# filodb/FiloDB

Measured on NVIDIA H100. Metric: samples/s scanned+aggregated (rate over 10M series); % HBM roofline, higher is better.
Workload: dtype f64

## Files before the change

### filodb_b200/csrc/capi.cu

```cuda
#include "../../include/filo_b200.h"
#include "kernels.h"
#include "host_util.h"
#include "scan_tile_layout.h"
#include "scan_wp_layout.h"
#include <cub/cub.cuh>
#include <algorithm>
#include <atomic>
#include <chrono>
#include <cmath>
#include <cstdio>
#include <cstdlib>
#include <cstring>
#include <mutex>
#include <string>
#include <thread>
#include <vector>

using namespace filo;

struct filo_ctx {
  int device = 0;
  filo_cfg cfg{};
  cudaStream_t stream = nullptr;
  int sm_count = 132;
// ... 799 lines not shown
  const uint32_t acc_bytes = fused ? align_up((uint32_t)q.T * (moments ? 20u : 12u), 128) : 0;
  const bool need_corr2 = need_corr && t->any_drop;
  uint32_t scratch2 = align_up((uint32_t)t->max_chunks * (uint32_t)CHUNK_DESC_BYTES, 16) +
                      ((uint32_t)t->max_rows + (uint32_t)t->max_chunks * 8u) * 8u * (1u + (t->any_nonconst_ts ? 1u : 0u) + (need_corr2 ? 1u : 0u));
  scratch2 = align_up(scratch2 + 16, 128);
  const uint32_t rec_cap = align_up(t->max_rec_bytes + 16, 128);
  const size_t per_warp2 = v2_smem_per_warp(rec_cap, scratch2, acc_bytes);
  const char* force_env = std::getenv("FILO_KERNEL");
  const std::string force = force_env ? force_env : "";
  const size_t smem_cap = std::min<size_t>(ctx->max_smem_optin, 227 * 1024);
  const bool use_v2 = force != "v1" && t->max_rec_bytes > 0 && per_warp2 * FAST_WARPS + 1024 <= smem_cap;
  const int64_t work = fused ? t->n_items : t->n_series;
  int64_t launches = 0;
  uint8_t* gscratch = nullptr;
  ScanLaunch L{t->d_arena, t->d_rec_off, t->n_series, q, nullptr, 0, 0, d_counters, d_err, 1, s};
  uint32_t rec_cap_used = 0;
  if (use_v2) {
    const size_t cta_smem = per_warp2 * FAST_WARPS + 1024;
    const int ctas_per_sm = (int)std::max<size_t>(1, std::min<size_t>(64 / FAST_WARPS, (size_t)(228 * 1024) / cta_smem));
    L.grid = (int)std::max<int64_t>(1, std::min<int64_t>((work + FAST_WARPS - 1) / FAST_WARPS, (int64_t)ctx->sm_count * ctas_per_sm));
    L.scratch_bytes = scratch2; L.use_smem = 1; rec_cap_used = rec_cap;
  } else {
    uint32_t scratch = align_up((uint32_t)t->max_chunks * (uint32_t)CHUNK_DESC_BYTES, 16) + (uint32_t)t->max_rows * 8u * (need_corr ? 3u : 2u);
    scratch = align_up(scratch + 16, 16);
    const size_t cta_smem = (size_t)(scratch + acc_bytes) * SCAN_WARPS;
    const int use_smem = cta_smem <= std::min<size_t>(ctx->max_smem_optin, 200 * 1024);
    int ctas_per_sm = 16;
    if (use_smem) ctas_per_sm = (int)std::max<size_t>(1, std::min<size_t>(16, (size_t)(220 * 1024) / std::max<size_t>(cta_smem + 1024, 1)));
    L.grid = (int)std::max<int64_t>(1, std::min<int64_t>((work + SCAN_WARPS - 1) / SCAN_WARPS, (int64_t)ctx->sm_count * ctas_per_sm));
    if (!use_smem) CUDA_TRY(ctx, tmp.alloc((void**)&gscratch, (size_t)L.grid * SCAN_WARPS * (scratch + acc_bytes)));
    L.gscratch = gscratch; L.scratch_bytes = scratch; L.use_smem = use_smem;
  }
  const int fn_cls = fn_class_of(fn, q.cumulative, q.long_values);
  const uint64_t wrows = (uint64_t)(q.window / q.step) + 1;
  TileSmem TL{};
  bool use_tile = false;
  if (use_v2 && force != "v2" && fn_cls == CLASS_SUM && t->n_series > 0) {
    TL = tile_layout(t->max_rec_bytes, (uint32_t)t->max_rows, (uint32_t)q.T, (uint32_t)std::min<uint64_t>(2 * wrows, 1u << 20) + 16);
    if (((size_t)TL.total + 1024) * 2 > (size_t)228 * 1024) TL = tile_layout(t->max_rec_bytes, (uint32_t)t->max_rows, (uint32_t)q.T, 16);
    use_tile = (size_t)TL.total + 1024 <= smem_cap;
  }
  WpSmem WL{};
  WpBatchSmem WB{};
  bool use_wp = false, use_wp_batch = false;
  if (use_tile && force != "v3" && wrows <= 4096 && t->max_chunks > 0) {
    const bool alias = wp_max_items((uint32_t)t->max_chunks, (uint32_t)q.T, (uint32_t)wrows) <= 64;
    WL = wp_layout(t->max_rec_bytes, (uint32_t)t->max_rows, (uint32_t)t->max_chunks, (uint32_t)q.T, (uint32_t)wrows, alias);
    WL.warps = (uint32_t)std::min<size_t>(smem_cap / WL.per_warp, alias ? WP_MAX_WARPS_ALIAS : WP_MAX_WARPS);
    const WpSmem WL2 = wp_layout(t->max_rec_bytes, (uint32_t)t->max_rows, (uint32_t)t->max_chunks, (uint32_t)q.T, (uint32_t)wrows, alias, true);
    if (smem_cap / WL2.per_warp >= (size_t)WP_MAX_WARPS) {
      WL = WL2; WL.warps = WP_MAX_WARPS;
      WB = wp_batch_layout(t->max_rec_bytes, (uint32_t)t->max_rows, (uint32_t)t->max_chunks, (uint32_t)q.T, (uint32_t)wrows, alias);
      use_wp_batch = WB.total <= smem_cap;
    }
    use_wp = WL.warps >= 4;
  }
  WpCtrSmem WC{};
  bool use_wp_ctr = false;
  if (use_v2 && force != "v2" && force != "v3" && fn_cls == CLASS_COUNTER && t->n_series > 0 && t->max_chunks > 0 &&
      (!fused || q.T <= TILE_AGG_ACC * TILE_THREADS) && wp_ctr_tile_footprint_ok(t->max_rec_bytes, (uint32_t)t->max_rows, (uint32_t)q.T, smem_cap)) {
    WC = wp_ctr_layout(t->max_rec_bytes, (uint32_t)t->max_rows, (uint32_t)t->max_chunks, (uint32_t)q.T, fused, t->any_nonconst_ts, moments);
    const size_t w = std::min<size_t>((smem_cap - sizeof(TileCtrTab) * (TILE_CTR_TABMAX + 1) - 64) / WC.per_warp, WC.tsr != 0 ? 16 : WP_CTR_MAX_WARPS);
    WC.warps = (uint32_t)w; WC.tab = (uint32_t)(WC.per_warp * w);
    use_wp_ctr = w >= 4;
  }
  auto run_per_series = [&](double* outp) -> int32_t {
    if (use_tile || use_wp_ctr) {
      int64_t* d_list = nullptr; unsigned long long* d_cnt = nullptr;
      CUDA_TRY(ctx, tmp.alloc((void**)&d_list, (size_t)t->n_series * 8));
      CUDA_TRY(ctx, tmp.alloc((void**)&d_cnt, 16));
      CUDA_TRY(ctx, cudaMemsetAsync(d_cnt, 0, 16, s));
      ScanLaunch LT = L;
      static const bool dbg = std::getenv("FILO_DEBUG_SYNC") != nullptr;
      if (use_wp_batch) {
        LT.grid = (int)std::max<int64_t>(1, std::min<int64_t>((t->n_series + WB.B - 1) / WB.B, (int64_t)ctx->sm_count));
        CUDA_TRY(ctx, launch_scan_wp_batch(LT, outp, WB, d_list, d_cnt));
      } else if (use_wp) {
        LT.grid = (int)std::max<int64_t>(1, std::min<int64_t>((t->n_series + WL.warps - 1) / WL.warps, (int64_t)ctx->sm_count));
        CUDA_TRY(ctx, launch_scan_wp(LT, outp, WL, d_list, d_cnt));
      } else if (use_wp_ctr) {
        LT.grid = (int)std::max<int64_t>(1, std::min<int64_t>((t->n_series + WC.warps - 1) / WC.warps, (int64_t)ctx->sm_count));
        CUDA_TRY(ctx, launch_scan_wp_ctr(LT, outp, WC, d_list, d_cnt));
      } else {
        const int ctas_per_sm = ((size_t)TL.total + 1024) * 2 <= (size_t)228 * 1024 ? 2 : 1;
        const int64_t n_tiles = (t->n_series + TILE_NS - 1) / TILE_NS;
        LT.grid = (int)std::max<int64_t>(1, std::min<int64_t>(n_tiles, (int64_t)ctx->sm_count * ctas_per_sm));
        if (dbg) { fprintf(stderr, "[filo] tile kernel fn=%d T=%d grid=%d smem=%u pitch=%u\n", fn, q.T, LT.grid, TL.total, TL.vals_pitch); fflush(stderr); }
        CUDA_TRY(ctx, launch_scan_tile(LT, outp, TL, d_list, d_cnt));
      }
      if (dbg) { CUDA_TRY(ctx, cudaStreamSynchronize(s)); fprintf(stderr, "[filo] tile kernel done\n"); fflush(stderr); }
      ScanLaunch LF = L; LF.list = d_list; LF.list_count = d_cnt;
      CUDA_TRY(ctx, launch_scan_series_v2(LF, outp, rec_cap_used));
      if (dbg) { CUDA_TRY(ctx, cudaStreamSynchronize(s)); fprintf(stderr, "[filo] fallback kernel done\n"); fflush(stderr); }
      launches += 2;
    } else {
      CUDA_TRY(ctx, use_v2 ? launch_scan_series_v2(L, outp, rec_cap_used) : launch_scan_series(L, outp));
      launches += 1;
    }
    return FILO_OK;
  };
  if (stats) CUDA_TRY(ctx, cudaEventRecord(e0, s));
  if (agg == FILO_AGG_NONE) {
    { int32_t rc = run_per_series((double*)d_out_values); if (rc) return rc; }
  } else if (!fused) {
    double* per = nullptr;
    CUDA_TRY(ctx, tmp.alloc((void**)&per, (size_t)t->n_series * q.T * 8));
// ... 559 lines not shown
```

### filodb_b200/csrc/scan_wp.cuh

```cuda
#pragma once
#include "scan_tile.cuh"
#include "scan_wp_layout.h"

namespace filo {

#ifdef FILO_CUSIM
__device__ __forceinline__ uint32_t wp_soff(const void* p) { return (uint32_t)(reinterpret_cast<const uint8_t*>(p) - smem); }
__device__ __forceinline__ uint32_t wp_lds32(uint32_t off) { uint32_t v; std::memcpy(&v, smem + off, 4); return v; }
#else
__device__ __forceinline__ uint32_t wp_soff(const void* p) { return smem_u32(p); }
__device__ __forceinline__ uint32_t wp_lds32(uint32_t off) { uint32_t v; asm volatile("ld.shared.u32 %0, [%1];" : "=r"(v) : "r"(off)); return v; }
#endif

#if defined(FILO_WP_PROF) && !defined(FILO_CUSIM)
__device__ unsigned long long g_wp_prof[32];
#define WPROF_DECL uint32_t wpp_t0 = (uint32_t)clock(), wpp_acc[14] = {0, 0, 0, 0, 0, 0, 0, 0, 0, 0, 0, 0, 0, 0};
#define WPROF(i) { const uint32_t wpp_t1 = (uint32_t)clock(); wpp_acc[i] += wpp_t1 - wpp_t0; wpp_t0 = wpp_t1; }
#define WPROF_COUNT(i) { ++wpp_acc[i]; }
#define WPROF_FLUSH if (lane == 0) { for (int wpp_i = 0; wpp_i < 14; ++wpp_i) atomicAdd(&g_wp_prof[wpp_i], (unsigned long long)wpp_acc[wpp_i]); atomicAdd(&g_wp_prof[15], 1ull); }
#else
#define WPROF_DECL
#define WPROF(i)
#define WPROF_COUNT(i)
#define WPROF_FLUSH
// ... 211 lines not shown
        TileDrops& D = DR[ci];
#pragma unroll
        for (int i = 0; i < 8; ++i) {
          const double cur = nan0(__longlong_as_double((long long)(d[jj][i] ^ pre)));
          if (i < nleft && cur < prevv) {
            const int at = atomicAdd(&D.n, 1);
            if (at < TILE_MAXDROP) { D.pos[at] = 1 + g * 8 + i; D.amt[at] = prevv; }
          }
          prevv = cur;
        }
      }
    }
  }
  for (int ci = 0; any_raw && ci < n; ++ci) {
    const WpChunk& ch = CD[ci];
    if (ch.wire != WIRE_RAW64) continue;
    const uint64_t* src = reinterpret_cast<const uint64_t*>(R + ch.val_off + 8);
    const bool drp = DROPS && ch.dropped;
    for (int r = lane; r < ch.nrows; r += 32) {
      const uint64_t b = src[r];
      reinterpret_cast<uint64_t*>(V)[wp_vidx(ch.rowpos + r)] = b;
      const uint32_t h = (uint32_t)(b >> 32);
      okbits &= h ^ (h << 1);
      if (drp && r > 0) {
        const double cur = nan0(__longlong_as_double((long long)b)), prevv = nan0(__longlong_as_double((long long)src[r - 1]));
        if (cur < prevv) { TileDrops& D = DR[ci]; const int at = atomicAdd(&D.n, 1); if (at < TILE_MAXDROP) { D.pos[at] = r; D.amt[at] = prevv; } }
      }
    }
  }
  if (any_raw) r_done();
  return okbits;
}

constexpr uint32_t WP_FINAL = 0, WP_RAWFIN = 1, WP_JUNC = 2, WP_GAP = 3;
__device__ __forceinline__ int wp_chunk_of(const WpChunk* CD, int n, int k) {
  int ci = -1;
  for (int c = 0; c < n; ++c) if (CD[c].nblk > 0 && k >= CD[c].kT0) ci = c;
  return ci;
}
__device__ __forceinline__ uint32_t wp_class(const WpChunk* CD, int n, int k, uint32_t& jslot) {
  const int ci = wp_chunk_of(CD, n, k);
  jslot = 0;
  if (ci < 0 || k > CD[ci].kT1) return WP_GAP;
  const WpChunk& ch = CD[ci];
  const int i = k - ch.kT0;
  if (i < ch.jzb * WP_R) { jslot = (uint32_t)(ch.joff + i) | (i < ch.hs ? 128u : 0u); return WP_JUNC; }
  return i >= ch.tb * WP_R ? WP_RAWFIN : WP_FINAL;
}
__device__ __forceinline__ int wp_rows_in(const WpChunk& x, int k, int Wr) {
  int lo = x.s0 + k; if (lo < 0) lo = 0; int hi = x.s0 + k + Wr; if (hi > x.nrows - 1) hi = x.nrows - 1;
  return hi - lo + 1;
}

__device__ __forceinline__ void wp_item(const WpChunk* CD, const WpSmem& L, int it, int items, int psi, int& pp, int& op, int& inf) {
  const bool active = it < items;
  int ci = 0;
  if (CD[1].nblk > 0 && it >= CD[1].blk0) ci = 1;
  if (CD[2].nblk > 0 && it >= CD[2].blk0) ci = 2;
  if (CD[3].nblk > 0 && it >= CD[3].blk0) ci = 3;
  const WpChunk& ch = CD[ci];
  const int b = active ? it - ch.blk0 : 0;
  const int k0 = ch.kT0 + WP_R * b;
  pp = ch.vidx0 + 9 * b;
  const bool tojz = b < ch.jzb;
  const bool raw = tojz || b >= ch.tb;
  op = tojz ? (int)WP_OFF_J + 8 * (ch.joff + WP_R * b) : (int)L.out + 8 * (k0 + ((k0 + psi) >> 3));
  int jEnd = !active ? -1 : tojz ? WP_R - 1 : ch.kT1 - k0;
  if (jEnd > WP_R - 1) jEnd = WP_R - 1;
  const int ot = tojz ? 0 : (k0 + psi) & 7;
  inf = (jEnd + 1) | ((raw ? 1 : 0) << 4) | (ot << 5) | (ci << 8) | (k0 << 10);
}

struct WpQuery {
  double fdiv, frcp;
  int64_t S0, E0, lastEnd;
  StepDiv sd;
  __device__ __forceinline__ void init(const QueryParams& q) {
    int64_t winDur = q.inclusive ? q.window : q.window - 1; if (winDur < 0) winDur = 0;
    fdiv = (double)(q.inclusive ? winDur : winDur + 1); frcp = 1.0 / fdiv;
    S0 = q.start - winDur; E0 = q.start;
    lastEnd = q.start + (int64_t)(q.T - 1) * q.step;
    sd.init(q.step);
  }
};
struct WpPlan {
  int64_t m_init = 0, m_end = 0; int m_nrows = -1, m_n = -1, m_wire = -1; bool m_ok = false;
  int dd_dst[2] = {0, 0}, dd_inf[2] = {0, 0}, wi_pp[2] = {0, 0}, wi_op[2] = {0, 0}, wi_inf[2] = {0, 0};
  int gz[3] = {-1, -1, -1}; bool gz_all = true;
  int p_Wr = 0, p_items = 0, p_nfull = 0, p_psi = 0; double p_rcpn = 0.0; bool p_oal = false;
  uint32_t p_cls = 0; uint64_t p_jx = 0;
};

__device__ __forceinline__ bool wp_plan_series(WpPlan& M, bool& regular, bool have, int n, int64_t init, int64_t end_time, int nrows, int vwire,
                                               int grp_base, int ngroups, const QueryParams& q, const WpSmem& L, const WpQuery& Q, WpChunk* CD, int lane) {
  const unsigned FULL = 0xffffffffu;
  const int c = lane;
  const bool samec = !(c < n) || (init == M.m_init && nrows == M.m_nrows && end_time == M.m_end && vwire == M.m_wire);
  const bool same_all = __all_sync(FULL, samec);
  const bool same = M.m_ok && n == M.m_n && same_all;
  const bool miss = regular && !same;
  if (miss) {
    M.m_init = init; M.m_end = end_time; M.m_nrows = nrows; M.m_n = n; M.m_wire = vwire; M.m_ok = false;
    int64_t s0 = 0, e0 = 0;
    if (have) { s0 = Q.sd.ceil_div(Q.S0 - init); e0 = Q.sd.floor_div(Q.E0 - init); }
    const int Wr = (int)(e0 - s0);
    int64_t kT0 = -e0; if (kT0 < 0) kT0 = 0;
    int64_t kT1 = (int64_t)(nrows - 1) - s0; if (kT1 > q.T - 1) kT1 = q.T - 1;
    const bool touch = have && kT0 <= kT1;
    if (!touch) { kT0 = 0x3fffffff; kT1 = -1; }
    const int Wr0 = __shfl_sync(FULL, Wr, 0);
    bool okp = !have || Wr == Wr0;
    if (Wr0 < 8 || (uint32_t)Wr0 + 1 > L.jcap) okp = false;
    const unsigned tm = __ballot_sync(FULL, touch) & 0xfu;
    if (tm != 0) { const unsigned lowbit = tm & (0u - tm); const unsigned filled = tm + lowbit; if ((filled & (filled - 1)) != 0) okp = false; }
    const int64_t kT1p = __shfl_up_sync(FULL, kT1, 1), kT1pp = __shfl_up_sync(FULL, kT1, 2), kT0n = __shfl_down_sync(FULL, kT0, 1);
    const bool prev_t = c > 0 && ((tm >> (c - 1)) & 1u), next_t = c + 1 < WP_MAXC && ((tm >> (c + 1)) & 1u);
    if (touch && c >= 2 && ((tm >> (c - 2)) & 1u) && !(kT1pp < kT0)) okp = false;
    int64_t ownLo = kT0, ownHi = kT1;
    if (touch && prev_t && kT1p + 1 > ownLo) ownLo = kT1p + 1;
    if (touch && next_t && kT0n - 1 < ownHi) ownHi = kT0n - 1;
    const int hs = touch ? (int)(ownLo - kT0) : 0;
    const int nblk = touch ? (int)((kT1 - kT0 + WP_R) / WP_R) : 0;
    const int jzb = (hs + WP_R - 1) / WP_R;
    const int tb = (touch && ownHi < kT1) ? (int)((ownHi + 1 - kT0) / WP_R) : nblk;
    if (touch && jzb > tb) okp = false;
    int blk0, items, joff, jtot;
    { const int a0 = __shfl_sync(FULL, nblk, 0), a1 = __shfl_sync(FULL, nblk, 1), a2 = __shfl_sync(FULL, nblk, 2), a3 = __shfl_sync(FULL, nblk, 3);
      blk0 = (c > 0 ? a0 : 0) + (c > 1 ? a1 : 0) + (c > 2 ? a2 : 0); items = a0 + a1 + a2 + a3; }
    { const int z = jzb * WP_R;
      const int a0 = __shfl_sync(FULL, z, 0), a1 = __shfl_sync(FULL, z, 1), a2 = __shfl_sync(FULL, z, 2), a3 = __shfl_sync(FULL, z, 3);
      joff = (c > 0 ? a0 : 0) + (c > 1 ? a1 : 0) + (c > 2 ? a2 : 0); jtot = a0 + a1 + a2 + a3; }
    if ((uint32_t)jtot > L.jcap) okp = false;
    if (L.alias && items > 64) okp = false;
    const int fr = touch ? (int)(s0 + kT0) : 0;
    int rowpos = 0;
    {
      int base = 0;
#pragma unroll
      for (int cc = 0; cc < WP_MAXC; ++cc) {
        int x;
        if (cc == 0) { x = fr < 0 ? -fr : ((8 - (fr & 7)) & 7); }
        else { x = base + ((-(base + fr)) & 7); }
        if (c == cc) rowpos = x;
        const int nb = __shfl_sync(FULL, x + nrows + Wr0, cc);
        base = nb;
      }
    }
    const int pend = __shfl_sync(FULL, rowpos + nrows, n > 0 ? n - 1 : 0) + Wr0 + 8;
    if ((uint32_t)(pend + (pend >> 3) + 2) > L.vcap) okp = false;
    if (!__all_sync(FULL, okp)) regular = false;
    if (regular) {
      if (c < WP_MAXC) {
        WpChunk& d = CD[c];
        d.kT0 = (int)kT0; d.kT1 = (int)kT1; d.ownLo = (int)ownLo; d.ownHi = (int)ownHi; d.blk0 = blk0; d.nblk = nblk;
        d.vidx0 = wp_vidx(rowpos + fr); d.rowpos = rowpos; d.nrows = nrows; d.s0 = (int)s0; d.e0 = (int)e0; d.joff = joff; d.hs = hs; d.jzb = jzb; d.tb = tb;
      }
      { const int first_t = tm ? __ffs((int)tm) - 1 : 0;
        M.p_psi = (-(int)__shfl_sync(FULL, (int)(touch ? kT0 : 0), first_t)) & 7;
        M.p_oal = __all_sync(FULL, !touch || (((int)kT0 + M.p_psi) & 7) == 0); }
      M.p_Wr = Wr0; M.p_items = items; M.p_nfull = Wr0 + 1; M.p_rcpn = 1.0 / (double)(Wr0 + 1);
      __syncwarp();
      {
        int tot = 0;
        M.gz[0] = M.gz[1] = M.gz[2] = -1;
        for (int g = 0; g <= n; ++g) {
          const int g0 = g == 0 ? 0 : CD[g - 1].rowpos + CD[g - 1].nrows;
          const int g1 = g == n ? pend : CD[g].rowpos;
#pragma unroll
          for (int u = 0; u < 3; ++u) { const int i = u * 32 + lane - tot; if (i >= 0 && i < g1 - g0) M.gz[u] = wp_vidx(g0 + i); }
          tot += g1 - g0;
        }
        M.gz_all = tot <= 96;
      }
      {
        uint32_t cls = 0; uint64_t jx = 0; int nj = 0;
#pragma unroll 1
        for (int m = 0; m < 16 && lane + 32 * m < q.T; ++m) {
          uint32_t js;
          const uint32_t code = wp_class(CD, n, lane + 32 * m, js);
          cls |= code << (2 * m);
          if (code == WP_JUNC) { jx |= (uint64_t)js << (8 * nj); ++nj; }
        }
        M.p_cls = cls; M.p_jx = jx;
      }
      {
        const int gb1 = __shfl_sync(FULL, have ? grp_base : 0x7fffffff, 1), gb2 = __shfl_sync(FULL, have ? grp_base : 0x7fffffff, 2),
                  gb3 = __shfl_sync(FULL, have ? grp_base : 0x7fffffff, 3);
#pragma unroll
        for (int jj = 0; jj < 2; ++jj) {
          const int slot = jj * 32 + lane;
          const bool active = slot < ngroups;
          const int ci = active ? (slot >= gb1 ? 1 : 0) + (slot >= gb2 ? 1 : 0) + (slot >= gb3 ? 1 : 0) : 0;
          const int gbc = ci == 0 ? 0 : ci == 1 ? gb1 : ci == 2 ? gb2 : gb3;
          const int g = active ? slot - gbc : 0;
          const int pq = CD[ci].rowpos + 1 + g * 8;
          M.dd_dst[jj] = wp_vidx(pq);
          M.dd_inf[jj] = (active ? 1 : 0) | (ci << 1) | ((pq & 7) << 3) | (g << 8);
        }
#pragma unroll
        for (int X = 0; X < 2; ++X) wp_item(CD, L, X * 32 + lane, items, M.p_psi, M.wi_pp[X], M.wi_op[X], M.wi_inf[X]);
      }
      M.m_ok = true;
    }
  }
  return miss;
}

__device__ __forceinline__ void wp_zero_rows(double* V, const WpChunk* CD, int n, const WpPlan& M, int lane) {
  if (M.gz_all) {
#pragma unroll
    for (int u = 0; u < 3; ++u) if (M.gz[u] >= 0) V[M.gz[u]] = 0.0;
  } else {
    const int pend = CD[n - 1].rowpos + CD[n - 1].nrows + M.p_Wr + 8;
    for (int g = 0; g <= n; ++g) {
      const int g0 = g == 0 ? 0 : CD[g - 1].rowpos + CD[g - 1].nrows;
      const int g1 = g == n ? pend : CD[g].rowpos;
      for (int pz = g0 + lane; pz < g1; pz += 32) V[wp_vidx(pz)] = 0.0;
    }
  }
}

template <int FN>
__device__ __forceinline__ void wp_window_blocks(const double* V, uint8_t* wb, const WpChunk* CD, const WpSmem& L, const WpPlan& M, const WpQuery& Q,
                                                 int lane) {
  const int psi = M.p_psi;
  const int Wr = M.p_Wr;
  for (int it0 = 0; it0 < M.p_items; it0 += 64) {
    int ipp[2], iop[2], iinf[2];
#pragma unroll
    for (int X = 0; X < 2; ++X) {
      if (it0 == 0) { ipp[X] = M.wi_pp[X]; iop[X] = M.wi_op[X]; iinf[X] = M.wi_inf[X]; }
      else wp_item(CD, L, it0 + X * 32 + lane, M.p_items, psi, ipp[X], iop[X], iinf[X]);
    }
    const double* pp[2]; double* op[2]; int jEnd[2], ot[2]; bool rawm[2];
#pragma unroll
    for (int X = 0; X < 2; ++X) {
      pp[X] = V + ipp[X]; op[X] = reinterpret_cast<double*>(wb + iop[X]);
      jEnd[X] = (iinf[X] & 15) - 1; rawm[X] = (iinf[X] >> 4) & 1; ot[X] = (iinf[X] >> 5) & 7;
    }
    double a[WP_R], bb[WP_R];
    wp_block_pair(pp[0], pp[1], Wr, a, bb);
    __syncwarp();
#pragma unroll
    for (int X = 0; X < 2; ++X) {
      const double dv = rawm[X] ? 1.0 : Q.fdiv, rc = rawm[X] ? 1.0 : Q.frcp, sc = rawm[X] ? 1.0 : 1000.0;
#pragma unroll
      for (int j = 0; j < WP_R; ++j) {
        const double raw = X ? bb[j] : a[j];
        int nn = 1;
        if (FN == FN_AVG || FN == FN_COUNT) {
          const WpChunk& ch = CD[(iinf[X] >> 8) & 3];
          int lo = ch.s0 + (iinf[X] >> 10) + j; const int hi0 = lo + Wr; if (lo < 0) lo = 0;
          const int hi = hi0 > ch.nrows - 1 ? ch.nrows - 1 : hi0;
          nn = hi - lo + 1;
        }
        const double fin = wp_finish<FN>(raw, nn, dv, rc, sc, M.p_nfull, M.p_rcpn, rawm[X]);
        if (X) bb[j] = fin; else a[j] = fin;
      }
    }
    if (M.p_oal) {
#pragma unroll
      for (int j = 0; j < WP_R; ++j) { if (j <= jEnd[0]) op[0][j] = a[j]; if (j <= jEnd[1]) op[1][j] = bb[j]; }
    } else {
#pragma unroll
      for (int j = 0; j < WP_R; ++j) {
        if (j <= jEnd[0]) op[0][j + ((ot[0] + j) >> 3)] = a[j];
        if (j <= jEnd[1]) op[1][j + ((ot[1] + j) >> 3)] = bb[j];
      }
    }
  }
  __syncwarp();
}

template <int FN, bool STAGE = false>
__device__ __forceinline__ void wp_finish_store(double* __restrict__ out, int64_t s, const QueryParams& q, double* O, const double* J,
                                                const WpChunk* CD, int n, const WpPlan& M, const WpQuery& Q, int lane) {
  const double NaNv = __longlong_as_double(0x7ff8000000000000LL);
  const int psi = M.p_psi, Wr = M.p_Wr;
  auto oidx = [&](int k) -> int { return k + ((k + psi) >> 3); };
  double* gp = out + (size_t)s * q.T + lane;
  const double* sp = O + oidx(lane);
  auto fin = [&](double o, uint32_t code, uint32_t js, int k) -> double {
    double v = o;
    if (code == WP_JUNC) { const double jv = J[js & 127u]; v = (js & 128u) ? o + jv : jv; }
    double r;
    if (FN == FN_COUNT) r = v;
    else {
      int nn = 1;
      if (FN == FN_AVG && (code == WP_RAWFIN || code == WP_JUNC)) {
        const int ci = wp_chunk_of(CD, n, k);
        nn = wp_rows_in(CD[ci], k, Wr);
        if (code == WP_JUNC && (js & 128u)) nn += wp_rows_in(CD[ci - 1], k, Wr);
      }
      r = wp_finish<FN>(v, nn, Q.fdiv, Q.frcp, 1000.0, M.p_nfull, M.p_rcpn, false);
    }
    return code == WP_FINAL ? o : code == WP_GAP ? NaNv : r;
  };
  uint32_t cls = M.p_cls; uint64_t jx = M.p_jx;
  auto fin_m = [&](double o, int k) -> double {
    const uint32_t code = cls & 3u, js = (uint32_t)jx & 0xffu;
    cls >>= 2;
    if (code == WP_JUNC) jx >>= 8;
    return fin(o, code, js, k);
  };
  if (STAGE) {
    const int T = q.T;
    double* row = out + (size_t)s * T;
    const int h = (int)((reinterpret_cast<uintptr_t>(row) >> 3) & 1);
    double* st = O + h + lane;
    int k = lane, iters = (T + 31) >> 5;
    int rest = iters > 16 ? iters - 16 : 0;
    if (rest) iters = 16;
    for (; iters >= 4; iters -= 4, st += 128, sp += 144, k += 128) {
      const bool in3 = k + 96 < T;
      const double v0 = sp[0], v1 = sp[36], v2 = sp[72], v3 = in3 ? sp[108] : 0.0;
      const double r0 = fin_m(v0, k), r1 = fin_m(v1, k + 32), r2 = fin_m(v2, k + 64), r3 = fin_m(v3, k + 96);
      __syncwarp();
      st[0] = r0; st[32] = r1; st[64] = r2; if (in3) st[96] = r3;
    }
    for (; iters > 0; --iters, st += 32, sp += 36, k += 32) {
      const bool in = k < T;
      const double r = fin_m(in ? *sp : 0.0, k);
      __syncwarp();
      if (in) *st = r;
    }
    for (; rest > 0; --rest, st += 32, sp += 36, k += 32) {
      const bool in = k < T;
      uint32_t js;
      const uint32_t code = wp_class(CD, n, k, js);
      const double r = fin(in ? *sp : 0.0, code, js, k);
      __syncwarp();
      if (in) *st = r;
    }
    fence_async_smem();
    __syncwarp();
    if (lane == 0) {
      const int nb = (T - h) & ~1;
      if (h) wp_store_result(row, O[1]);
      if ((T - h) & 1) wp_store_result(row + T - 1, O[T - 1 + h]);
      if (nb > 0) tma_store_1d(row + h, O + 2 * h, (uint32_t)nb * 8u);
    }
    return;
  }
  int k = lane, iters = (q.T - lane + 31) >> 5;
  int rest = iters > 16 ? iters - 16 : 0;
  if (rest) iters = 16;
  for (; iters >= 4; iters -= 4, gp += 128, sp += 144, k += 128) {
    const double v0 = sp[0], v1 = sp[36], v2 = sp[72], v3 = sp[108];
    const double r0 = fin_m(v0, k), r1 = fin_m(v1, k + 32), r2 = fin_m(v2, k + 64), r3 = fin_m(v3, k + 96);
    wp_store_result(gp, r0); wp_store_result(gp + 32, r1); wp_store_result(gp + 64, r2); wp_store_result(gp + 96, r3);
  }
  for (; iters > 0; --iters, gp += 32, sp += 36, k += 32) wp_store_result(gp, fin_m(*sp, k));
  for (; rest > 0; --rest, gp += 32, sp += 36, k += 32) {
    uint32_t js;
    const uint32_t code = wp_class(CD, n, k, js);
    wp_store_result(gp, fin(*sp, code, js, k));
  }
}
__device__ __forceinline__ void wp_stage_wait(int lane) {
  if (lane == 0) tma_store_wait_read();
  __syncwarp();
}

__device__ __forceinline__ void wp_series_desc(WpChunk* CD, int c, bool have, int grp_base, int ng, int vwire, uint32_t voff, int dropped, uint64_t first,
                                               uint32_t grp_off, uint32_t tab_off) {
  if (c < WP_MAXC) {
    WpChunk& d = CD[c];
    d.grp_base = have ? grp_base : 0x7fffffff; d.ng = ng; d.wire = vwire; d.val_off = voff; d.dropped = dropped;
    d.first = first; d.grp_off = grp_off; d.tab_off = tab_off;
  }
}

template <int FN, int NW>
__global__ void __launch_bounds__(NW * 32, 1)
scan_wp_sum_kernel(const uint8_t* __restrict__ arena, const int64_t* __restrict__ rec_off, int64_t n_series, QueryParams q,
                   double* __restrict__ out, WpSmem L, int64_t* __restrict__ fallback_list, unsigned long long* __restrict__ fallback_count,
                   unsigned long long* d_counters, int* d_err) {
  extern __shared__ __align__(128) uint8_t smem[];
  const unsigned FULL = 0xffffffffu;
  const int lane = threadIdx.x & 31, warp = threadIdx.x >> 5;
  uint8_t* wb = smem + (size_t)warp * L.per_warp;
  uint64_t* bar = reinterpret_cast<uint64_t*>(wb);
  WpChunk* CD = reinterpret_cast<WpChunk*>(wb + WP_OFF_DESC);
  uint64_t* xtab = reinterpret_cast<uint64_t*>(wb + WP_OFF_J);
  double* J = reinterpret_cast<double*>(wb + WP_OFF_J);
// ... 226 lines not shown
          WpEntryChunk& ec = e.c[c];
          ec.first = first; ec.init = init; ec.end_time = end_time; ec.grp_off = grp_off; ec.val_off = voff;
          ec.nrows = nrows; ec.grp_base = grp_base; ec.ng = ng; ec.wire = (uint32_t)vwire | ((uint32_t)dropped << 16);
          if (c == 0) {
            e.rofs = rofs; e.n = n; e.flags = (regular ? 1 : 0) | (any_raw ? 2 : 0); e.ngroups = a0 + a1 + a2 + a3;
            e.cnt_rows = cnt_rows; e.cnt_bytes = cnt_bytes;
          }
        }
      }
      __syncwarp();
      if (lane == 0) mbar_arrive(parsed + b);
      WPPROD(2)
      WPPROD_COUNT
    }
    WPPROD_FLUSH
    return;
  }

  uint8_t* wb = smem + (size_t)warp * L.per_warp;
  WpChunk* CD = reinterpret_cast<WpChunk*>(wb + WP_OFF_DESC);
  uint64_t* xtab = reinterpret_cast<uint64_t*>(wb + WP_OFF_J);
  double* J = reinterpret_cast<double*>(wb + WP_OFF_J);
  double* V = reinterpret_cast<double*>(wb + L.vals);
  double* O = reinterpret_cast<double*>(wb + L.out);
  const int c = lane;
  WpQuery Q; Q.init(q);
  WpPlan M;
  int64_t rows_scanned = 0, bytes_scanned = 0;
  int i = warp / B, slot = warp % B;
  WPROF_DECL
  for (;; slot += NC) {
    while (slot >= B) { slot -= B; ++i; }
    const int64_t s = ((int64_t)blockIdx.x + (int64_t)i * gridDim.x) * B + slot;
    if (s >= n_series) break;
    const int b = i % NB, u = i / NB;
    WPROF_COUNT(10)
    WPROF(9)
    mbar_wait(parsed + b, u & 1);
    mbar_wait(full + b, u & 1);
    WPROF(0)
    const WpEntry& e = ENT[(size_t)b * B + slot];
    const uint8_t* R = smem + BL.buf + (size_t)b * BL.buf_stride + e.rofs;
    const int n = e.n, flags = e.flags;
    bool regular = flags & 1;
    const bool have = regular && c < n;
    int64_t init = 0, end_time = 0; int nrows = 0, grp_base = 0, ng = 0, wire = 0; uint32_t voff = 0, grp_off = 0; uint64_t first = 0;
    if (c < WP_MAXC) {
      const WpEntryChunk& ec = e.c[c];
      init = ec.init; end_time = ec.end_time; nrows = ec.nrows; grp_base = ec.grp_base; ng = ec.ng; wire = (int)ec.wire;
      voff = ec.val_off; grp_off = ec.grp_off; first = ec.first;
    }
    const int vwire = wire & 0xffff;
    WPROF(1)
    if (wp_plan_series(M, regular, have, n, init, end_time, nrows, vwire, grp_base, e.ngroups, q, L, Q, CD, lane)) { WPROF_COUNT(11) }
    WPROF(2)
    if (!regular) {
      WPROF_COUNT(12)
      __syncwarp();
      if (lane == 0) {
        const unsigned long long fs = atomicAdd(fallback_count, 1ull); fallback_list[fs] = s;
        mbar_arrive(empty + b);
      }
      __syncwarp();
      continue;
    }
    wp_series_desc(CD, c, have, grp_base, ng, vwire, voff, wire >> 16, first, grp_off, have && vwire == WIRE_XOR ? voff + XOR_OFF_GROUPTAB : 0u);
    const int cnt_rows = e.cnt_rows, cnt_bytes = e.cnt_bytes;
    const bool any_raw = (flags & 2) != 0;
    __syncwarp();
    WPROF(3)
    wp_stage_wait(lane);
    WPROF(8)
    auto rec_done = [&]() {
      __syncwarp();
      if (lane == 0) mbar_arrive(empty + b);
    };
    const uint32_t okbits = wp_decode<false>(R, V, CD, xtab, M.dd_dst, M.dd_inf, n, any_raw, lane, nullptr, rec_done);
    const bool vals_ok = __all_sync(FULL, (okbits >> 30) & 1u);
    __syncwarp();
    WPROF(4)
    wp_zero_rows(V, CD, n, M, lane);
    WPROF(5)
    if (!vals_ok) {
      WPROF_COUNT(13)
      if (lane == 0) { const unsigned long long fs = atomicAdd(fallback_count, 1ull); fallback_list[fs] = s; }
      __syncwarp();
      continue;
    }
    if (lane == 0) { rows_scanned += cnt_rows; bytes_scanned += cnt_bytes; }
    __syncwarp();
    wp_window_blocks<FN>(V, wb, CD, L, M, Q, lane);
    WPROF(6)
    wp_finish_store<FN, true>(out, s, q, O, J, CD, n, M, Q, lane);
    __syncwarp();
    WPROF(7)
  }
  WPROF(9)
  WPROF_FLUSH
  if (lane == 0) {
    tma_store_wait_all();
    if (rows_scanned | bytes_scanned) { atomicAdd(&d_counters[0], (unsigned long long)rows_scanned); atomicAdd(&d_counters[1], (unsigned long long)bytes_scanned); }
  }
}

}
```

### filodb_b200/csrc/scan_wp_layout.h

```cpp
#pragma once
#include <stdint.h>
#include "filo_record.h"
#include "scan_params.h"
#include "scan_tile_layout.h"
namespace filo {
constexpr int WP_MAXC = 4;
constexpr int WP_MAXG = 64;
constexpr int WP_R = 8;
constexpr int WP_MAX_WARPS = 16;
constexpr int WP_MAX_WARPS_ALIAS = 20;

struct WpChunk {
  uint64_t first;
  int32_t kT0, kT1;
  int32_t ownLo, ownHi;
  int32_t blk0, nblk;
  int32_t vidx0;
  int32_t rowpos;
  int32_t nrows, s0, e0;
  int32_t grp_base, ng, wire;
  uint32_t grp_off, tab_off, val_off;
  int32_t joff, hs;
  int32_t jzb, tb;
  int32_t dropped;
// ... 9 lines not shown
  uint32_t rec2;
};
FILO_HD inline WpSmem wp_layout(uint32_t max_rec_bytes, uint32_t max_rows, uint32_t max_chunks, uint32_t T, uint32_t wrows, bool alias, bool two_rec = false) {
  WpSmem L;
  if (max_chunks > (uint32_t)WP_MAXC) max_chunks = WP_MAXC;
  L.rec_cap = align_up(max_rec_bytes + 16, 16);
  const uint32_t P = max_rows + (max_chunks + 1) * (wrows + 7) + 16;
  L.vcap = align_up(P + P / 8 + 2, 2);
  L.jcap = WP_J_DOUBLES;
  (void)wrows;
  L.ocap = align_up(T + T / 8 + 4, 2);
  if (alias && L.vcap < L.ocap) L.vcap = L.ocap;
  static_assert(sizeof(WpChunk) == 96, "WP_OFF_J");
  uint32_t o = WP_OFF_REC;
  L.desc = WP_OFF_DESC; L.jbuf = WP_OFF_J;
  L.rec = o; o += L.rec_cap;
  L.rec2 = 0;
  if (two_rec) { L.rec2 = o; o += L.rec_cap; }
  L.vals = o; o += L.vcap * 8;
  if (alias) L.out = L.vals; else { L.out = o; o += L.ocap * 8; }
  L.per_warp = align_up(o, 16);
  L.warps = 0;
  L.alias = alias ? 1u : 0u;
  return L;
}

constexpr int WP_BATCH_WARPS = 16;
constexpr int WP_BATCH_SERIES = 15;
constexpr int WP_BATCH_BUFS = 2;
struct WpEntryChunk {
  uint64_t first;
  int64_t init, end_time;
  uint32_t grp_off, val_off;
  int32_t nrows, grp_base, ng;
  uint32_t wire;
};
static_assert(sizeof(WpEntryChunk) == 48, "WpEntryChunk");
struct WpEntry {
  uint32_t rofs;
  int32_t n;
  int32_t flags;
  int32_t ngroups, cnt_rows, cnt_bytes;
  int32_t pad[2];
  WpEntryChunk c[WP_MAXC];
};
static_assert(sizeof(WpEntry) == 224, "WpEntry");
struct WpBatchSmem {
  WpSmem W;
  uint32_t B, nbuf, consumers;
  uint32_t buf, buf_stride, buf_cap;
  uint32_t ent;
  uint32_t bars;
  uint32_t total;
};
FILO_HD inline WpBatchSmem wp_batch_layout(uint32_t max_rec_bytes, uint32_t max_rows, uint32_t max_chunks, uint32_t T, uint32_t wrows, bool alias,
                                           uint32_t B = WP_BATCH_SERIES, uint32_t nbuf = WP_BATCH_BUFS, uint32_t consumers = WP_BATCH_WARPS - 1) {
  WpBatchSmem S;
  WpSmem L = wp_layout(max_rec_bytes, max_rows, max_chunks, T, wrows, alias);
  const uint32_t shift = L.vals - WP_OFF_REC;
  L.vals -= shift; L.out -= shift; L.per_warp -= shift; L.rec = 0;
  S.consumers = consumers;
  L.warps = S.consumers;
  S.W = L; S.B = B; S.nbuf = nbuf;
  uint32_t o = L.per_warp * S.consumers;
  S.buf = o;
  S.buf_cap = B * align_up(max_rec_bytes, 16);
  S.buf_stride = S.buf_cap + 16;
  o += nbuf * S.buf_stride;
  S.ent = o; o += nbuf * B * (uint32_t)sizeof(WpEntry);
  S.bars = o; o += 3 * nbuf * 8;
  S.total = align_up(o, 16);
  return S;
}

FILO_HD inline uint32_t wp_max_items(uint32_t max_chunks, uint32_t T, uint32_t wrows) {
  if (max_chunks > (uint32_t)WP_MAXC) max_chunks = WP_MAXC;
  if (max_chunks == 0) max_chunks = 1;
  return (T + (max_chunks - 1) * (wrows - 1) + 7 * max_chunks) / 8;
}

constexpr int WP_CTR_MAX_WARPS = 20;
struct TileCtr {
  double dTS, thr, half, endpart, sI, ratio0, skipC;
  int32_t dropped, pad;
};
constexpr int TILE_MAXDROP = 8;
constexpr int TILE_CTR_TABMAX = 64;
struct TileCtrTab { double sI, thr, half, rcpSI; };
struct TileDrops {
  int32_t n, pos[TILE_MAXDROP], pad[3];
  double amt[TILE_MAXDROP];
};
struct WpCtrChunk {
  int64_t init, end_time;
  int32_t nrows, s0, e0, rowpos;
  int32_t kA, kB;
  int32_t kA2, kB2;
  TileCtr kc;
};
static_assert(sizeof(WpCtrChunk) == 112, "WpCtrChunk");

struct WpCtrSmem {
  uint32_t vals, kc, acc, nbad, per_warp, tab ;
  uint32_t rec_cap, vcap , warps, agg;
  uint32_t tsr;
};
constexpr uint32_t WP_OFF_DROPS = WP_OFF_J + 64 * 8;
static_assert(WP_OFF_DROPS + WP_MAXC * sizeof(TileDrops) <= WP_OFF_REC, "drops fit in front of the record");
FILO_HD inline WpCtrSmem wp_ctr_layout(uint32_t max_rec_bytes, uint32_t max_rows, uint32_t max_chunks, uint32_t T, bool agg, bool irr = false,
                                       bool moments = false) {
  WpCtrSmem L;
  if (max_chunks > (uint32_t)WP_MAXC) max_chunks = WP_MAXC;
  L.rec_cap = align_up(max_rec_bytes + 16, 16);
// ... 22 lines not shown
```

### scratch/wp_prof.py

```python
import ctypes as C
import os
import sys

import numpy as np

HERE = os.path.dirname(os.path.abspath(__file__))
sys.path.insert(0, os.path.dirname(HERE))
import filodb_b200.capi as capi
capi.LIB_PATH = os.environ.get("FILO_LIB_PATH") or os.path.join(HERE, "libfilo_b200_wp_prof.so")
import bench

workload = sys.argv[1] if len(sys.argv) > 1 else "c2"
series = sys.argv[2] if len(sys.argv) > 2 else "5000000"
L = capi.lib()
L.filo_debug_wp_prof.argtypes = [C.c_void_p, C.c_int]
out = np.zeros(32, np.uint64)
sys.argv = ["bench.py", "--workload", workload, "--series", series, "--steps", "4", "--warmup", "2", "--no-e2e", "--no-cpu", "--no-extra", "--no-c5"]
L.filo_debug_wp_prof(out.ctypes.data, 1)
bench.main()
L.filo_debug_wp_prof(out.ctypes.data, 0)
names = ["wait: record (mbarrier)", "parse", "memo check (+ window plan on a miss)", "per-series descriptors, scan counters", "decode",
         "zero rows", "window blocks", "finish and store (earlier: fix-up, gaps)", "wait: previous row's bulk store", "loop head, declined series"]
ns = float(out[10])
tot = float(out[:10].sum())
print("SUM kernel: %d consumer warps, %d series taken up, %d memo misses, %d declined by the plan, %d declined by the values"
      % (int(out[15]), int(ns), int(out[11]), int(out[12]), int(out[13])))
print("  %-40s %10s %7s" % ("phase", "cyc/series", "share"))
for i, n in enumerate(names):
    if i == 8 and out[i] == 0:
        continue
    print("  %-40s %10.1f %6.1f %%" % (n, float(out[i]) / ns, 100.0 * float(out[i]) / tot))
print("  %-40s %10.1f" % ("total", tot / ns))
if out[20]:
    nb = float(out[19])
    ptot = float(out[16:19].sum())
    print("producer: %d warps, %d batches" % (int(out[20]), int(nb)))
    for i, n in enumerate(["stalled on the empty barrier", "offsets, copy issue, copy wait", "header parse, entries"]):
        print("  %-40s %10.1f %6.1f %%" % (n, float(out[16 + i]) / nb, 100.0 * float(out[16 + i]) / ptot))
    print("  %-40s %10.1f" % ("total", ptot / nb))
```

Before: 165.5 billion.

## Write finished window blocks directly into the staged output row in batch kernel

In the batch WP kernel, window blocks that need no fix-up are now written straight into the staging row at the output's alignment offset. Raw tail blocks go to a new per-warp tail region. The finish pass then only patches raw, junction and tail positions, using the class bitmask, instead of re-reading and re-finishing every element of the padded buffer. This removes a full smem read-and-rewrite pass per series. In exchange it adds a lane-rotation shuffle on stores, extra per-warp shared memory for tails, a plan reject when the tails overflow, and a new unsupported-error path for aliased multi-pass plans.

```diff
diff --git a/filodb_b200/csrc/capi.cu b/filodb_b200/csrc/capi.cu
--- a/filodb_b200/csrc/capi.cu
+++ b/filodb_b200/csrc/capi.cu
@@ -875,6 +875,8 @@
       WL = WL2; WL.warps = WP_MAX_WARPS;
       WB = wp_batch_layout(t->max_rec_bytes, (uint32_t)t->max_rows, (uint32_t)t->max_chunks, (uint32_t)q.T, (uint32_t)wrows, alias);
       use_wp_batch = WB.total <= smem_cap;
+      if (use_wp_batch && WB.W.alias && wp_max_items((uint32_t)t->max_chunks, (uint32_t)q.T, (uint32_t)wrows) > 64)
+        return fail(ctx, FILO_ERR_UNSUPPORTED, "scan_wp_batch_kernel: O on V with plans of more than one pass");
     }
     use_wp = WL.warps >= 4;
   }
diff --git a/filodb_b200/csrc/scan_wp.cuh b/filodb_b200/csrc/scan_wp.cuh
--- a/filodb_b200/csrc/scan_wp.cuh
+++ b/filodb_b200/csrc/scan_wp.cuh
@@ -287,7 +287,15 @@
   return hi - lo + 1;
 }
 
-__device__ __forceinline__ void wp_item(const WpChunk* CD, const WpSmem& L, int it, int items, int psi, int& pp, int& op, int& inf) {
+__device__ __forceinline__ int wp_tail_base(const WpChunk* CD, int c) {
+  int t = 0;
+#pragma unroll
+  for (int x = 0; x < WP_MAXC - 1; ++x) if (x < c) t += CD[x].nblk - CD[x].tb;
+  return WP_R * t;
+}
+
+template <bool STAGE = false>
+__device__ __forceinline__ void wp_item(const WpChunk* CD, const WpSmem& L, int it, int items, int psi, int& pp, int& op, int& inf, uint32_t rt = 0) {
   const bool active = it < items;
   int ci = 0;
   if (CD[1].nblk > 0 && it >= CD[1].blk0) ci = 1;
@@ -299,10 +307,11 @@
   pp = ch.vidx0 + 9 * b;
   const bool tojz = b < ch.jzb;
   const bool raw = tojz || b >= ch.tb;
-  op = tojz ? (int)WP_OFF_J + 8 * (ch.joff + WP_R * b) : (int)L.out + 8 * (k0 + ((k0 + psi) >> 3));
+  if (STAGE) op = tojz ? (int)WP_OFF_J + 8 * (ch.joff + WP_R * b) : b >= ch.tb ? (int)rt + 8 * (wp_tail_base(CD, ci) + WP_R * (b - ch.tb)) : (int)L.out + 8 * k0;
+  else op = tojz ? (int)WP_OFF_J + 8 * (ch.joff + WP_R * b) : (int)L.out + 8 * (k0 + ((k0 + psi) >> 3));
   int jEnd = !active ? -1 : tojz ? WP_R - 1 : ch.kT1 - k0;
   if (jEnd > WP_R - 1) jEnd = WP_R - 1;
-  const int ot = tojz ? 0 : (k0 + psi) & 7;
+  const int ot = tojz || STAGE ? 0 : (k0 + psi) & 7;
   inf = (jEnd + 1) | ((raw ? 1 : 0) << 4) | (ot << 5) | (ci << 8) | (k0 << 10);
 }
 
@@ -326,8 +335,10 @@
   uint32_t p_cls = 0; uint64_t p_jx = 0;
 };
 
+template <bool STAGE = false>
 __device__ __forceinline__ bool wp_plan_series(WpPlan& M, bool& regular, bool have, int n, int64_t init, int64_t end_time, int nrows, int vwire,
-                                               int grp_base, int ngroups, const QueryParams& q, const WpSmem& L, const WpQuery& Q, WpChunk* CD, int lane) {
+                                               int grp_base, int ngroups, const QueryParams& q, const WpSmem& L, const WpQuery& Q, WpChunk* CD, int lane,
+                                               uint32_t rt = 0, uint32_t rtcap = 0) {
   const unsigned FULL = 0xffffffffu;
   const int c = lane;
   const bool samec = !(c < n) || (init == M.m_init && nrows == M.m_nrows && end_time == M.m_end && vwire == M.m_wire);
@@ -366,6 +377,11 @@
       const int a0 = __shfl_sync(FULL, z, 0), a1 = __shfl_sync(FULL, z, 1), a2 = __shfl_sync(FULL, z, 2), a3 = __shfl_sync(FULL, z, 3);
       joff = (c > 0 ? a0 : 0) + (c > 1 ? a1 : 0) + (c > 2 ? a2 : 0); jtot = a0 + a1 + a2 + a3; }
     if ((uint32_t)jtot > L.jcap) okp = false;
+    if (STAGE) {
+      const int t = nblk - tb;
+      const int a0 = __shfl_sync(FULL, t, 0), a1 = __shfl_sync(FULL, t, 1), a2 = __shfl_sync(FULL, t, 2);
+      if ((uint32_t)(WP_R * (a0 + a1 + a2)) > rtcap) okp = false;
+    }
     if (L.alias && items > 64) okp = false;
     const int fr = touch ? (int)(s0 + kT0) : 0;
     int rowpos = 0;
@@ -433,7 +449,7 @@
           M.dd_inf[jj] = (active ? 1 : 0) | (ci << 1) | ((pq & 7) << 3) | (g << 8);
         }
 #pragma unroll
-        for (int X = 0; X < 2; ++X) wp_item(CD, L, X * 32 + lane, items, M.p_psi, M.wi_pp[X], M.wi_op[X], M.wi_inf[X]);
+        for (int X = 0; X < 2; ++X) wp_item<STAGE>(CD, L, X * 32 + lane, items, M.p_psi, M.wi_pp[X], M.wi_op[X], M.wi_inf[X], rt);
       }
       M.m_ok = true;
     }
@@ -455,9 +471,9 @@
   }
 }
 
-template <int FN>
+template <int FN, bool STAGE = false>
 __device__ __forceinline__ void wp_window_blocks(const double* V, uint8_t* wb, const WpChunk* CD, const WpSmem& L, const WpPlan& M, const WpQuery& Q,
-                                                 int lane) {
+                                                 int lane, int h = 0, uint32_t rt = 0) {
   const int psi = M.p_psi;
   const int Wr = M.p_Wr;
   for (int it0 = 0; it0 < M.p_items; it0 += 64) {
@@ -465,13 +481,14 @@
 #pragma unroll
     for (int X = 0; X < 2; ++X) {
       if (it0 == 0) { ipp[X] = M.wi_pp[X]; iop[X] = M.wi_op[X]; iinf[X] = M.wi_inf[X]; }
-      else wp_item(CD, L, it0 + X * 32 + lane, M.p_items, psi, ipp[X], iop[X], iinf[X]);
+      else wp_item<STAGE>(CD, L, it0 + X * 32 + lane, M.p_items, psi, ipp[X], iop[X], iinf[X], rt);
     }
     const double* pp[2]; double* op[2]; int jEnd[2], ot[2]; bool rawm[2];
 #pragma unroll
     for (int X = 0; X < 2; ++X) {
       pp[X] = V + ipp[X]; op[X] = reinterpret_cast<double*>(wb + iop[X]);
       jEnd[X] = (iinf[X] & 15) - 1; rawm[X] = (iinf[X] >> 4) & 1; ot[X] = (iinf[X] >> 5) & 7;
+      if (STAGE && !rawm[X]) op[X] += h;
     }
     double a[WP_R], bb[WP_R];
     wp_block_pair(pp[0], pp[1], Wr, a, bb);
@@ -493,7 +510,20 @@
         if (X) bb[j] = fin; else a[j] = fin;
       }
     }
-    if (M.p_oal) {
+    if (STAGE) {
+      const int r = 4 * ((lane >> 1) & 1);
+#pragma unroll
+      for (int X = 0; X < 2; ++X) {
+        double (&v)[WP_R] = X ? bb : a;
+        double t[WP_R];
+#pragma unroll
+        for (int j = 0; j < WP_R; ++j) t[j] = r ? v[(j + 4) & 7] : v[j];
+#pragma unroll
+        for (int j = 0; j < WP_R; ++j) v[j] = t[j];
+#pragma unroll
+        for (int j = 0; j < WP_R; ++j) { const int sj = (j + r) & 7; if (sj <= jEnd[X]) op[X][sj] = v[j]; }
+      }
+    } else if (M.p_oal) {
 #pragma unroll
       for (int j = 0; j < WP_R; ++j) { if (j <= jEnd[0]) op[0][j] = a[j]; if (j <= jEnd[1]) op[1][j] = bb[j]; }
     } else {
@@ -509,7 +539,8 @@
 
 template <int FN, bool STAGE = false>
 __device__ __forceinline__ void wp_finish_store(double* __restrict__ out, int64_t s, const QueryParams& q, double* O, const double* J,
-                                                const WpChunk* CD, int n, const WpPlan& M, const WpQuery& Q, int lane) {
+                                                const WpChunk* CD, int n, const WpPlan& M, const WpQuery& Q, int lane, const double* RT = nullptr,
+                                                int h = 0) {
   const double NaNv = __longlong_as_double(0x7ff8000000000000LL);
   const int psi = M.p_psi, Wr = M.p_Wr;
   auto oidx = [&](int k) -> int { return k + ((k + psi) >> 3); };
@@ -541,31 +572,26 @@
   if (STAGE) {
     const int T = q.T;
     double* row = out + (size_t)s * T;
-    const int h = (int)((reinterpret_cast<uintptr_t>(row) >> 3) & 1);
-    double* st = O + h + lane;
-    int k = lane, iters = (T + 31) >> 5;
-    int rest = iters > 16 ? iters - 16 : 0;
-    if (rest) iters = 16;
-    for (; iters >= 4; iters -= 4, st += 128, sp += 144, k += 128) {
-      const bool in3 = k + 96 < T;
-      const double v0 = sp[0], v1 = sp[36], v2 = sp[72], v3 = in3 ? sp[108] : 0.0;
-      const double r0 = fin_m(v0, k), r1 = fin_m(v1, k + 32), r2 = fin_m(v2, k + 64), r3 = fin_m(v3, k + 96);
-      __syncwarp();
-      st[0] = r0; st[32] = r1; st[64] = r2; if (in3) st[96] = r3;
-    }
-    for (; iters > 0; --iters, st += 32, sp += 36, k += 32) {
-      const bool in = k < T;
-      const double r = fin_m(in ? *sp : 0.0, k);
-      __syncwarp();
-      if (in) *st = r;
-    }
-    for (; rest > 0; --rest, st += 32, sp += 36, k += 32) {
-      const bool in = k < T;
+    auto tail = [&](int c, int k) -> double { return RT[wp_tail_base(CD, c) + k - CD[c].kT0 - WP_R * CD[c].tb]; };
+    auto fix = [&](uint32_t code, uint32_t js, int k) {
+      double o = 0.0;
+      if (code == WP_RAWFIN) o = tail(wp_chunk_of(CD, n, k), k);
+      else if (code == WP_JUNC && (js & 128u)) o = tail(wp_chunk_of(CD, n, k) - 1, k);
+      O[k + h] = fin(o, code, js, k);
+    };
+    uint32_t nf = (cls | (cls >> 1)) & 0x55555555u;
+    while (nf) {
+      const int b = __ffs((int)nf) - 1;
+      nf &= nf - 1;
+      const uint32_t code = (cls >> b) & 3u;
+      uint32_t js = 0;
+      if (code == WP_JUNC) { js = (uint32_t)jx & 0xffu; jx >>= 8; }
+      fix(code, js, lane + 16 * b);
+    }
+    for (int k = lane + 512; k < T; k += 32) {
       uint32_t js;
       const uint32_t code = wp_class(CD, n, k, js);
-      const double r = fin(in ? *sp : 0.0, code, js, k);
-      __syncwarp();
-      if (in) *st = r;
+      if (code != WP_FINAL) fix(code, js, k);
     }
     fence_async_smem();
     __syncwarp();
@@ -898,7 +924,7 @@
     }
     const int vwire = wire & 0xffff;
     WPROF(1)
-    if (wp_plan_series(M, regular, have, n, init, end_time, nrows, vwire, grp_base, e.ngroups, q, L, Q, CD, lane)) { WPROF_COUNT(11) }
+    if (wp_plan_series<true>(M, regular, have, n, init, end_time, nrows, vwire, grp_base, e.ngroups, q, L, Q, CD, lane, BL.rt, BL.rtcap)) { WPROF_COUNT(11) }
     WPROF(2)
     if (!regular) {
       WPROF_COUNT(12)
@@ -935,9 +961,10 @@
     }
     if (lane == 0) { rows_scanned += cnt_rows; bytes_scanned += cnt_bytes; }
     __syncwarp();
-    wp_window_blocks<FN>(V, wb, CD, L, M, Q, lane);
+    const int h = (int)((reinterpret_cast<uintptr_t>(out + s * q.T) >> 3) & 1);
+    wp_window_blocks<FN, true>(V, wb, CD, L, M, Q, lane, h, BL.rt);
     WPROF(6)
-    wp_finish_store<FN, true>(out, s, q, O, J, CD, n, M, Q, lane);
+    wp_finish_store<FN, true>(out, s, q, O, J, CD, n, M, Q, lane, reinterpret_cast<const double*>(wb + BL.rt), h);
     __syncwarp();
     WPROF(7)
   }
diff --git a/filodb_b200/csrc/scan_wp_layout.h b/filodb_b200/csrc/scan_wp_layout.h
--- a/filodb_b200/csrc/scan_wp_layout.h
+++ b/filodb_b200/csrc/scan_wp_layout.h
@@ -85,6 +85,7 @@
   uint32_t ent;
   uint32_t bars;
   uint32_t total;
+  uint32_t rt, rtcap;
 };
 FILO_HD inline WpBatchSmem wp_batch_layout(uint32_t max_rec_bytes, uint32_t max_rows, uint32_t max_chunks, uint32_t T, uint32_t wrows, bool alias,
                                            uint32_t B = WP_BATCH_SERIES, uint32_t nbuf = WP_BATCH_BUFS, uint32_t consumers = WP_BATCH_WARPS - 1) {
@@ -92,6 +93,11 @@
   WpSmem L = wp_layout(max_rec_bytes, max_rows, max_chunks, T, wrows, alias);
   const uint32_t shift = L.vals - WP_OFF_REC;
   L.vals -= shift; L.out -= shift; L.per_warp -= shift; L.rec = 0;
+  const uint32_t mc = max_chunks < (uint32_t)WP_MAXC ? max_chunks : (uint32_t)WP_MAXC;
+  S.rtcap = mc > 1 ? (uint32_t)WP_R * (mc - 1) * ((wrows + 14) / 8) : 0;
+  S.rt = L.out + 8 * (T + 1);
+  { const uint32_t oreg = alias ? L.vcap : L.ocap, need = T + 1 + S.rtcap;
+    L.per_warp = align_up(L.out + 8 * (oreg > need ? oreg : need), 16); }
   S.consumers = consumers;
   L.warps = S.consumers;
   S.W = L; S.B = B; S.nbuf = nbuf;
diff --git a/scratch/wp_prof.py b/scratch/wp_prof.py
--- a/scratch/wp_prof.py
+++ b/scratch/wp_prof.py
@@ -20,7 +20,7 @@
 bench.main()
 L.filo_debug_wp_prof(out.ctypes.data, 0)
 names = ["wait: record (mbarrier)", "parse", "memo check (+ window plan on a miss)", "per-series descriptors, scan counters", "decode",
-         "zero rows", "window blocks", "finish and store (earlier: fix-up, gaps)", "wait: previous row's bulk store", "loop head, declined series"]
+         "zero rows", "window blocks", "finish and store (batch kernel: fix-up and store)", "wait: previous row's bulk store", "loop head, declined series"]
 ns = float(out[10])
 tot = float(out[:10].sum())
 print("SUM kernel: %d consumer warps, %d series taken up, %d memo misses, %d declined by the plan, %d declined by the values"
```

After: 174.8 billion (median of 6 runs). 5.6% higher.
